# bharatlytics/faceRecognition_InfrenceEngine

Measured on AMD Instinct MI355X. Metric: faces/sec end-to-end @1080p, higher is better.
Workload: dtype f16

## Files before the change

### facerecognition_infrenceengine_amd/csrc/pnet_conv1.hip

```cpp
#include "detect_math.h"

namespace {

struct P1Args {
    const uint8_t* frames; int B, FH, FW;
    int H, W;
    const float* w;
    const float* bias; const float* slope;
    float* y;
    unsigned char* y_split;
    int Ho, Wo, Hp, Wp, regions_x, regions_y;
    const int32_t* list; const int32_t* list_count; int list_cap;
};

constexpr int P1_TW = 64, P1_IW = P1_TW + 2;
constexpr int P1_OCC = 3;
constexpr int P1_CTU = 4;
constexpr int P1_LEVEL_SHIFT = 27, P1_TILE_MASK = (1 << P1_LEVEL_SHIFT) - 1;

__device__ __forceinline__ float dpp_xor1(float v) {
    return __int_as_float(__builtin_amdgcn_update_dpp(0, __float_as_int(v), 0xB1, 0xf, 0xf, true));
}
__device__ __forceinline__ float dpp_shr1(float v) {
    return __int_as_float(__builtin_amdgcn_update_dpp(0, __float_as_int(v), 0x111, 0xf, 0xf, true));
}

template <int RPW, int RPB, bool F16, bool LIST>
__device__ __forceinline__ void pnet_conv1_body(const P1Args& a, const int item0, const int nitems) {
    constexpr int TH = 4 * RPW, IH = TH + 2, NPX = IH * P1_IW;
    constexpr int NPF = (NPX + 255) / 256;
    constexpr int NTAB = IH + P1_IW;
    constexpr int XPX = NPF * 256;
    static_assert(!F16 || XPX >= NPX + P1_IW + 4, "slack behind the tile for the zero-weight taps");
    constexpr int NXB = RPB > 1 ? 2 : 1, NTB = RPB > 1 ? 3 : 1;
    constexpr int XFL = F16 ? XPX * 4 : XPX * 3;
    __shared__ __attribute__((aligned(16))) float xin2[NXB][XFL];
    __shared__ __attribute__((aligned(16))) int4v tab[NTB][NTAB];
    const int tid = threadIdx.x, lane = tid & 63, wave = tid >> 6;
    const float pinf = opaque_inf();

    float wreg[6];
    half8 wfh[2], wfl[2];
    if constexpr (F16) {
#pragma unroll
        for (int st = 0; st < 2; ++st)
#pragma unroll
            for (int j = 0; j < 8; ++j) {
                const int kq_ = lane >> 4, kh = 2 * st + (kq_ >> 1), kw = (kq_ & 1) * 2 + (j >> 2), c = j & 3;
                const float w = (kh < 3 && kw < 3 && c < 3) ? a.w[((kh * 3 + kw) * 4 + c) * 16 + (lane & 15)] : 0.f;
                split_f16(w, wfh[st], wfl[st], j);
            }
    } else {
#pragma unroll
    for (int v = 0; v < 6; ++v) {
        const int c = v * 16 + (lane >> 2), r = lane & 3;
        float x = 0.f;
        if (c < 81) {
            const int k = c / 3, g = c - k * 3, tap = k / 3, ch = k - tap * 3;
            x = a.w[(tap * 4 + ch) * 16 + g * 4 + r];
        }
        wreg[v] = x;
    }
    }

    const int per_img = a.regions_x * a.regions_y;
    auto tile_of = [&](int item) { return LIST ? a.list[item] & P1_TILE_MASK : item; };
    const float ryr = (float)a.FH / (float)a.H, rxr = (float)a.FW / (float)a.W;
    const int frame_bytes = a.FH * a.FW * 3;

    auto make_tables = [&](int item, int buf) __attribute__((always_inline)) {
        if (tid < NTAB) {
            const int tile = tile_of(item);
            const int n = tile / per_img, rem = tile - n * per_img;
            const int ry = rem / a.regions_x, rx = rem - ry * a.regions_x;
            int4v e;
            if (tid < IH) {
                const int yy = ry * TH + tid;
                const Lerp l = lerp_coord(yy, ryr, a.FH);
                e = int4v{l.i0 * a.FW * 3, l.i1 * a.FW * 3, __float_as_int(l.w), yy < a.H ? 1 : 0};
            } else {
                const int xx = rx * P1_TW + (tid - IH);
                const Lerp l = lerp_coord(xx, rxr, a.FW);
                e = int4v{l.i0 * 3, __float_as_int(l.w), l.i1 != l.i0 ? 1 : 0, xx < a.W ? 1 : 0};
            }
            tab[buf][tid] = e;
        }
    };

    unsigned long long rq0[NPF], rq1[NPF];
    int rfl[NPF];
    int pos[NPF];
#pragma unroll
    for (int u = 0; u < NPF; ++u) {
        const int e = min(tid + u * 256, NPX - 1), iy = e / P1_IW;
        pos[u] = iy | ((IH + e - iy * P1_IW) << 16);
    }
    bool edge = true;
    auto load_tile = [&](int item, int buf) __attribute__((always_inline)) {
        const int n = tile_of(item) / per_img;
        const uint8_t* fbase = a.frames + (int64_t)n * frame_bytes;
        const bool last = n == a.B - 1;
        const int lim = frame_bytes - 8;
        int4v re[NPF], ce[NPF];
        bool special = false;
#pragma unroll
        for (int u = 0; u < NPF; ++u) { re[u] = tab[buf][pos[u] & 0xffff]; ce[u] = tab[buf][pos[u] >> 16]; }
#pragma unroll
        for (int u = 0; u < NPF; ++u) {
            const bool valid = (re[u][3] & ce[u][3]) != 0;
            const int o0 = valid ? re[u][0] + ce[u][0] : 0, o1 = valid ? re[u][1] + ce[u][0] : 0;
            int c0 = o0, c1 = o1, fl = ce[u][2];
            if (last) {
                c0 = min(o0, lim); c1 = min(o1, lim);
                fl |= ((o0 - c0) << 11) | ((o1 - c1) << 19);
            }
            rq0[u] = *reinterpret_cast<const u64_unaligned*>(fbase + c0);
            rq1[u] = *reinterpret_cast<const u64_unaligned*>(fbase + c1);
            rfl[u] = valid ? fl : -1;
            special = special || !valid || !(fl & 1);
        }
        edge = last || __builtin_amdgcn_ballot_w64(special) != 0;
    };
    auto store_tile_as = [&](int buf, float* xin, auto EDGE) __attribute__((always_inline)) {
        constexpr bool E = decltype(EDGE)::value;
        float wy[NPF], wx[NPF];
#pragma unroll
        for (int u = 0; u < NPF; ++u) {
            wy[u] = __int_as_float(tab[buf][pos[u] & 0xffff][2]);
            wx[u] = __int_as_float(tab[buf][pos[u] >> 16][1]);
        }
#pragma unroll
        for (int u = 0; u < NPF; ++u) {
            const int e = tid + u * 256;
            float v[3];
            const unsigned long long q0 = E ? rq0[u] >> ((rfl[u] >> 8) & 0xff) : rq0[u];
            const unsigned long long q1 = E ? rq1[u] >> ((rfl[u] >> 16) & 0xff) : rq1[u];
            const unsigned l0 = (unsigned)q0, h0 = (unsigned)(q0 >> 32), l1 = (unsigned)q1, h1 = (unsigned)(q1 >> 32);
            const bool two = !E || (rfl[u] & 1) != 0;
            const float a00[3] = {(float)((l0 >> 16) & 0xff), (float)((l0 >> 8) & 0xff), (float)(l0 & 0xff)};
            const float a01[3] = {(float)((h0 >> 8) & 0xff), (float)(h0 & 0xff), (float)(l0 >> 24)};
            const float a10[3] = {(float)((l1 >> 16) & 0xff), (float)((l1 >> 8) & 0xff), (float)(l1 & 0xff)};
            const float a11[3] = {(float)((h1 >> 8) & 0xff), (float)(h1 & 0xff), (float)(l1 >> 24)};
#pragma unroll
            for (int c = 0; c < 3; ++c) {
                const float sv = bilerp(a00[c], two ? a01[c] : a00[c], a10[c], two ? a11[c] : a10[c], wx[u], wy[u]);
                v[c] = (!E || rfl[u] >= 0) ? __builtin_fmaf(sv, 0.0078125f, -0.99609375f) : 0.f;
            }
            if constexpr (F16) {
                half4 hi, lo;
#pragma unroll
                for (int c = 0; c < 3; ++c) split_f16(v[c], hi, lo, c);
                hi[3] = lo[3] = (half_t)0.f;
                unsigned char* xz = reinterpret_cast<unsigned char*>(xin);
                *reinterpret_cast<half4*>(xz + e * 8) = hi;
                *reinterpret_cast<half4*>(xz + (XPX + e) * 8) = lo;
            } else {
                xin[e * 3 + 0] = v[0]; xin[e * 3 + 1] = v[1]; xin[e * 3 + 2] = v[2];
            }
        }
    };
    auto store_tile = [&](int buf, float* xdst) __attribute__((always_inline)) {
        if (edge) store_tile_as(buf, xdst, std::true_type{});
        else store_tile_as(buf, xdst, std::false_type{});
    };

    float4v bias_r[3], slope_r[3];
    bool mono = true;
#pragma unroll
    for (int g = 0; g < 3; ++g) {
        bias_r[g] = *reinterpret_cast<const float4v*>(a.bias + g * 4);
        slope_r[g] = *reinterpret_cast<const float4v*>(a.slope + g * 4);
#pragma unroll
        for (int e = 0; e < 4; ++e) mono = mono && slope_r[g][e] >= 0.f;
    }
    if (item0 < nitems) {
        make_tables(item0, 0);
        __syncthreads();
        load_tile(item0, 0);
        if (RPB > 1 && item0 + 1 < nitems) make_tables(item0 + 1, 1);
        if (RPB > 2 && item0 + 2 < nitems) make_tables(item0 + 2, 2);
        store_tile(0, xin2[0]);
    }
    __syncthreads();
    if (RPB > 1 && item0 + 1 < nitems) load_tile(item0 + 1, 1);

    for (int rr = 0; rr < RPB; ++rr) {
        const int item = item0 + rr;
        if (item >= nitems) break;
        const int tile_ = tile_of(item);
        const int n = tile_ / per_img, rem = tile_ - n * per_img;
        const int ry = rem / a.regions_x, rx = rem - ry * a.regions_x;
        const int y0 = ry * TH, x0 = rx * P1_TW;
        const float* xin = xin2[rr & (NXB - 1)];
        if constexpr (RPB > 1) {
            if (rr + 1 < RPB && item + 1 < nitems) store_tile((rr + 1) % 3, xin2[(rr + 1) & 1]);
            if (rr + 2 < RPB && item + 2 < nitems) load_tile(item + 2, (rr + 2) % 3);
            if (rr + 3 < RPB && item + 3 < nitems) make_tables(item + 3, rr % 3);
        }

        if constexpr (F16) {
            typedef half8 half8_a8 __attribute__((aligned(8)));
            const unsigned char* xz = reinterpret_cast<const unsigned char*>(xin);
            const int li = lane & 15, kq = lane >> 4;
            const float4v b4 = *reinterpret_cast<const float4v*>(a.bias + 4 * kq), s4 = *reinterpret_cast<const float4v*>(a.slope + 4 * kq);
            const int64_t fbase = (int64_t)n * a.Hp;
            auto conv16 = [&](int row, int ct) __attribute__((always_inline)) {
                const unsigned char* pb = xz + ((row + (kq >> 1)) * P1_IW + ct * 16 + li + 2 * (kq & 1)) * 8;
                const half8 h0 = *reinterpret_cast<const half8_a8*>(pb), l0 = *reinterpret_cast<const half8_a8*>(pb + XPX * 8);
                const half8 h1 = *reinterpret_cast<const half8_a8*>(pb + 2 * P1_IW * 8), l1 = *reinterpret_cast<const half8_a8*>(pb + (XPX + 2 * P1_IW) * 8);
                float4v q = {0.f, 0.f, 0.f, 0.f};
                q = __builtin_amdgcn_mfma_f32_16x16x32_f16(wfl[0], h0, q, 0, 0, 0);
                q = __builtin_amdgcn_mfma_f32_16x16x32_f16(wfh[0], l0, q, 0, 0, 0);
                q = __builtin_amdgcn_mfma_f32_16x16x32_f16(wfl[1], h1, q, 0, 0, 0);
                q = __builtin_amdgcn_mfma_f32_16x16x32_f16(wfh[1], l1, q, 0, 0, 0);
                q = __builtin_amdgcn_mfma_f32_16x16x32_f16(wfh[0], h0, q, 0, 0, 0);
                q = __builtin_amdgcn_mfma_f32_16x16x32_f16(wfh[1], h1, q, 0, 0, 0);
                return q;
            };
            auto put16 = [&](const float4v& m, int py, int px) __attribute__((always_inline)) {
                const int64_t pix = (fbase + py) * a.Wp + px;
                half4 hi, lo;
#pragma unroll
                for (int e = 0; e < 4; ++e) split_f16(m[e], hi, lo, e);
                const int2v hp = __builtin_bit_cast(int2v, hi), lp = __builtin_bit_cast(int2v, lo);
                const auto s0 = __builtin_amdgcn_permlane16_swap((unsigned)hp[0], (unsigned)lp[0], false, false);
                const auto s1 = __builtin_amdgcn_permlane16_swap((unsigned)hp[1], (unsigned)lp[1], false, false);
                *reinterpret_cast<int4v*>(a.y_split + pix * 64 + (kq & 1) * 32 + (kq >> 1) * 16) = int4v{(int)s0[0], (int)s1[0], (int)s0[1], (int)s1[1]};
                if (a.y && kq < 3) *reinterpret_cast<float4v*>(a.y + pix * 12 + 4 * kq) = m;
            };
            if (mono) {
                static_assert(RPW == 4 || !F16, "the packed epilogue pairs the wave's two row pairs");
                const bool interior = y0 + TH <= a.Ho && x0 + P1_TW <= a.Wo;
                float4v s4m, b4z;
#pragma unroll
                for (int e = 0; e < 4; ++e) { s4m[e] = 4 * kq + e < 10 ? s4[e] - 1.f : -1.f; b4z[e] = 4 * kq + e < 10 ? b4[e] : 0.f; }
                const int odd = li & 1;
                const int py = ((y0 + wave * RPW) >> 1) + odd;
#pragma unroll P1_CTU
                for (int ct = 0; ct < 4; ++ct) {
                    float4v m[2];
#pragma unroll
                    for (int rp = 0; rp < 2; ++rp) {
                        float4v d0 = conv16(wave * RPW + 2 * rp, ct), d1 = conv16(wave * RPW + 2 * rp + 1, ct);
                        if (!interior) {
                            const bool cin = x0 + ct * 16 + li < a.Wo;
                            const bool in0 = cin && y0 + wave * RPW + 2 * rp < a.Ho, in1 = cin && y0 + wave * RPW + 2 * rp + 1 < a.Ho;
#pragma unroll
                            for (int e = 0; e < 4; ++e) { d0[e] = in0 ? d0[e] : -INFINITY; d1[e] = in1 ? d1[e] : -INFINITY; }
                        }
#pragma unroll
                        for (int e = 0; e < 4; ++e) {
                            const float t = vmax(d0[e], d1[e], pinf);
                            m[rp][e] = vmax(t, dpp_xor1(t), pinf);
                        }
                    }
                    float4v v;
#pragma unroll
                    for (int e = 0; e < 4; ++e) {
                        float sh = dpp_shr1(m[1][e]);
                        asm volatile("" : "+v"(sh));
                        const float x = (odd ? sh : m[0][e]) + b4z[e];
                        v[e] = __builtin_fmaf(fminf(x, 0.f), s4m[e], x);
                    }
                    const int px = ((x0 + ct * 16) >> 1) + (li >> 1);
                    if (py < a.Hp && px < a.Wp) put16(v, py, px);
                }
            } else {
#pragma unroll
            for (int rp = 0; rp < RPW / 2; ++rp) {
#pragma unroll
                for (int ct = 0; ct < 4; ++ct) {
                    float4v d[2];
#pragma unroll
                    for (int h = 0; h < 2; ++h) {
                        const int row = wave * RPW + 2 * rp + h;
                        float4v q = conv16(row, ct);
                        q += b4;
#pragma unroll
                        for (int e = 0; e < 4; ++e) q[e] = q[e] > 0.f ? q[e] : q[e] * s4[e];
                        const bool inside = y0 + row < a.Ho && x0 + ct * 16 + li < a.Wo;
                        d[h] = inside ? q : float4v{-INFINITY, -INFINITY, -INFINITY, -INFINITY};
                    }
                    float4v m;
#pragma unroll
                    for (int e = 0; e < 4; ++e) {
                        const float t = vmax(d[0][e], d[1][e], pinf);
                        m[e] = 4 * kq + e < 10 ? vmax(t, dpp_xor1(t), pinf) : 0.f;
                    }
                    const int py = (y0 + wave * RPW + 2 * rp) >> 1, px = (x0 + ct * 16 + li) >> 1;
                    if ((li & 1) == 0 && py < a.Hp && px < a.Wp) put16(m, py, px);
                }
            }
            }
        } else {
        float4v acc[RPW][3];
#pragma unroll
        for (int r = 0; r < RPW; ++r)
#pragma unroll
            for (int g = 0; g < 3; ++g) acc[r][g] = float4v{0.f, 0.f, 0.f, 0.f};
        const float* xb = xin + ((wave * RPW) * P1_IW + lane) * 3;
        static_for<RPW + 2>([&](auto IR) {
            constexpr int ir = decltype(IR)::value;
            float xv[9];
#pragma unroll
            for (int q = 0; q < 9; ++q) xv[q] = xb[ir * P1_IW * 3 + q];
            static_for<9>([&](auto Q) {
                constexpr int q = decltype(Q)::value;
                static_for<3>([&](auto KH) {
                    constexpr int kh = decltype(KH)::value, r = ir - kh;
                    if constexpr (r >= 0 && r < RPW) {
                        static_for<3>([&](auto G) {
                            constexpr int g = decltype(G)::value;
                            constexpr int c = (kh * 9 + q) * 3 + g;
                            acc[r][g] = __builtin_amdgcn_mfma_f32_4x4x1f32(wreg[c / 16], xv[q], acc[r][g], 4, c % 16, 0);
                        });
                    }
                });
            });
        });

        const int xcol = x0 + lane;
        const bool interior = y0 + TH <= a.Ho && x0 + P1_TW <= a.Wo;
        auto put = [&](const float4v (&pv)[3], int py, int px) __attribute__((always_inline)) {
            const int64_t pix = ((int64_t)n * a.Hp + py) * a.Wp + px;
            float* o = a.y + pix * 12;
#pragma unroll
            for (int g = 0; g < 3; ++g) *reinterpret_cast<float4v*>(o + g * 4) = pv[g];
            if (a.y_split) {
                half8 hi[2], lo[2];
#pragma unroll
                for (int c = 0; c < 16; ++c) split_f16(c < 10 ? pv[c >> 2][c & 3] : 0.f, hi[c >> 3], lo[c >> 3], c & 7);
                unsigned char* o2 = a.y_split + pix * 64;
                *reinterpret_cast<half8*>(o2) = hi[0];
                *reinterpret_cast<half8*>(o2 + 16) = hi[1];
                *reinterpret_cast<half8*>(o2 + 32) = lo[0];
                *reinterpret_cast<half8*>(o2 + 48) = lo[1];
            }
        };
        if (mono) {
            if (!interior) {
#pragma unroll
                for (int r = 0; r < RPW; ++r) {
                    const bool inside = y0 + wave * RPW + r < a.Ho && xcol < a.Wo;
#pragma unroll
                    for (int g = 0; g < 3; ++g)
                        acc[r][g] = inside ? acc[r][g] : float4v{-INFINITY, -INFINITY, -INFINITY, -INFINITY};
                }
            }
            float4v pv[RPW / 2][3];
#pragma unroll
            for (int rp = 0; rp < RPW / 2; ++rp)
#pragma unroll
                for (int g = 0; g < 3; ++g)
#pragma unroll
                    for (int e = 0; e < 4; ++e) {
                        const float m = vmax(acc[2 * rp][g][e], acc[2 * rp + 1][g][e], pinf);
                        pv[rp][g][e] = vmax(m, dpp_xor1(m), pinf);
                    }
            float4v q[3];
            int py = (y0 + wave * RPW) >> 1;
            bool writer = (lane & 1) == 0;
            if constexpr (RPW == 4) {
#pragma unroll
                for (int g = 0; g < 3; ++g)
#pragma unroll
                    for (int e = 0; e < 4; ++e) {
                        const float t = dpp_shr1(pv[1][g][e]);
                        q[g][e] = (lane & 1) ? t : pv[0][g][e];
                    }
                py += lane & 1;
                writer = true;
            } else {
#pragma unroll
                for (int g = 0; g < 3; ++g) q[g] = pv[0][g];
            }
#pragma unroll
            for (int g = 0; g < 3; ++g) {
                q[g] += bias_r[g];
#pragma unroll
                for (int e = 0; e < 4; ++e) q[g][e] = q[g][e] > 0.f ? q[g][e] : q[g][e] * slope_r[g][e];
            }
            const int px = (x0 >> 1) + (lane >> 1);
            if (writer && py < a.Hp && px < a.Wp) put(q, py, px);
        } else {
#pragma unroll
            for (int r = 0; r < RPW; ++r) {
                const bool inside = y0 + wave * RPW + r < a.Ho && xcol < a.Wo;
#pragma unroll
                for (int g = 0; g < 3; ++g) {
                    float4v v = acc[r][g] + bias_r[g];
#pragma unroll
                    for (int e = 0; e < 4; ++e) v[e] = v[e] > 0.f ? v[e] : v[e] * slope_r[g][e];
                    acc[r][g] = inside ? v : float4v{-INFINITY, -INFINITY, -INFINITY, -INFINITY};
                }
            }
#pragma unroll
            for (int rp = 0; rp < RPW / 2; ++rp) {
                float4v pv[3];
#pragma unroll
                for (int g = 0; g < 3; ++g)
#pragma unroll
                    for (int e = 0; e < 4; ++e) {
                        const float m = vmax(acc[2 * rp][g][e], acc[2 * rp + 1][g][e], pinf);
                        pv[g][e] = vmax(m, dpp_xor1(m), pinf);
                    }
                const int py = (y0 + wave * RPW + 2 * rp) >> 1, px = xcol >> 1;
                if ((lane & 1) == 0 && py < a.Hp && px < a.Wp) put(pv, py, px);
            }
        }
        }
        if (rr + 1 < RPB && item + 1 < nitems) __syncthreads();
    }
}

template <int RPW, int RPB, bool F16 = false, bool LIST = false>
__global__ __launch_bounds__(256, RPW == 4 ? (F16 ? P1_OCC : 3) : 6) void pnet_conv1_kernel(P1Args a) {
    const int nitems = LIST ? min(*a.list_count, a.list_cap) : a.regions_x * a.regions_y * a.B;
    pnet_conv1_body<RPW, RPB, F16, LIST>(a, blockIdx.x * RPB, nitems);
}

#define P1_MAXL 16
struct P1Levels {
    float* y[P1_MAXL]; unsigned char* y_split[P1_MAXL];
    int H[P1_MAXL], W[P1_MAXL], rpb[P1_MAXL], first[P1_MAXL + 1];
    int nlevels;
};
template <int RPW, int RPB, bool F16 = false, bool LIST = false>
__global__ __launch_bounds__(256, RPW == 4 ? (F16 ? P1_OCC : 3) : 6) void pnet_conv1_levels(P1Args a, P1Levels t) {
    int l = 0, item0 = blockIdx.x, nitems = 0;
    if constexpr (LIST) {
        if (item0 >= min(*a.list_count, a.list_cap)) return;
        l = min((int)((unsigned)a.list[item0] >> P1_LEVEL_SHIFT), t.nlevels - 1);
        nitems = item0 + 1;
    } else {
        while (l + 1 < t.nlevels && (int)blockIdx.x >= t.first[l + 1]) ++l;
    }
    a.H = t.H[l]; a.W = t.W[l]; a.y = t.y[l]; a.y_split = t.y_split[l];
    a.Ho = a.H - 2; a.Wo = a.W - 2; a.Hp = (a.Ho + 1) / 2; a.Wp = (a.Wo + 1) / 2;
    a.regions_x = (a.Wo + P1_TW - 1) / P1_TW; a.regions_y = (a.Ho + 4 * RPW - 1) / (4 * RPW);
    if constexpr (!LIST) {
        item0 = ((int)blockIdx.x - t.first[l]) * t.rpb[l];
        nitems = min(a.regions_x * a.regions_y * a.B, item0 + t.rpb[l]);
    }
    pnet_conv1_body<RPW, RPB, F16, LIST>(a, item0, nitems);
}

template <int RPW, int RPB, bool F16 = false, bool LIST = false>
int launch_p1(P1Args a, hipStream_t s) {
    constexpr int TH = 4 * RPW;
    a.regions_x = (a.Wo + P1_TW - 1) / P1_TW;
    a.regions_y = (a.Ho + TH - 1) / TH;
    const int64_t nitems = LIST ? a.list_cap : (int64_t)a.regions_x * a.regions_y * a.B;
    if (nitems >= (LIST ? 1ll << P1_LEVEL_SHIFT : 1ll << 31)) return FR_E_INVALID;
    pnet_conv1_kernel<RPW, RPB, F16, LIST><<<(unsigned)((nitems + RPB - 1) / RPB), 256, 0, s>>>(a);
    return FR_OK;
}

}

int fr_pnet_conv1_launch(const uint8_t* frames, int B, int FH, int FW, int H, int W, const float* w, const float* bias,
                         const float* slope, float* y, void* y_split, hipStream_t s) {
    P1Args a{frames, B, FH, FW, H, W, w, bias, slope, y, (unsigned char*)y_split, H - 2, W - 2, 0, 0, 0, 0, nullptr, nullptr, 0};
    a.Hp = (a.Ho + 1) / 2; a.Wp = (a.Wo + 1) / 2;
    const int64_t tiles16 = (int64_t)((a.Ho + 15) / 16) * ((a.Wo + P1_TW - 1) / P1_TW) * B;
    if (tiles16 >= 4096) return launch_p1<4, 8>(a, s);
    if (tiles16 >= 512) return launch_p1<4, 1>(a, s);
    return launch_p1<2, 1>(a, s);
}

extern "C" int fr_pnet_conv1_band(int mode, const uint8_t* frames, int B, int FH, int FW, int H, int W, const float* w,
                                  const float* bias, const float* slope, float* y, void* y_split, const int32_t* list,
                                  const int32_t* list_count, int list_cap, fr_stream_t stream) {
    FR_REQUIRE(frames && w && bias && slope && B > 0 && FH > 0 && FW > 0 && H >= 3 && W >= 3, "fr_pnet_conv1_band: bad argument");
    P1Args a{frames, B, FH, FW, H, W, w, bias, slope, y, (unsigned char*)y_split, H - 2, W - 2, 0, 0, 0, 0, list, list_count, list_cap};
    a.Hp = (a.Ho + 1) / 2; a.Wp = (a.Wo + 1) / 2;
    hipStream_t s = fr_stream(stream);
    int rc;
    if (mode == 0) {
        FR_REQUIRE(y_split, "fr_pnet_conv1_band: mode 0 writes the split map");
        const int64_t tiles16 = (int64_t)((a.Ho + 15) / 16) * ((a.Wo + P1_TW - 1) / P1_TW) * B;
        rc = tiles16 >= 4096 ? launch_p1<4, 8, true>(a, s) : launch_p1<4, 1, true>(a, s);
    } else if (mode == 1) {
        FR_REQUIRE(y && list && list_count && list_cap > 0, "fr_pnet_conv1_band: mode 1 needs the f32 map and a tile list");
        rc = launch_p1<4, 1, false, true>(a, s);
    } else { FR_REQUIRE(false, "fr_pnet_conv1_band: mode must be 0 or 1"); }
    if (rc != FR_OK) { fr_set_error("fr_pnet_conv1_band: too many tiles"); return rc; }
    FR_CHECK_LAUNCH("pnet_conv1_kernel (band)");
    return FR_OK;
}

extern "C" int fr_pnet_pyramid_conv1(int mode, const uint8_t* frames, int B, int FH, int FW, const fr_pnet_level* levels, int nlevels,
                                     const float* w, const float* bias, const float* slope, const int32_t* list,
                                     const int32_t* list_count, int list_cap, fr_stream_t stream) {
    FR_REQUIRE(frames && w && bias && slope && levels && B > 0 && FH > 0 && FW > 0 && nlevels > 0 && nlevels <= P1_MAXL,
               "fr_pnet_pyramid_conv1: bad argument (1 .. %d levels)", P1_MAXL);
    FR_REQUIRE(mode == 0 || mode == 1, "fr_pnet_pyramid_conv1: mode must be 0 or 1");
    for (int l = 0; l < nlevels; ++l) {
        const fr_pnet_level& L = levels[l];
        FR_REQUIRE(L.x1 && L.x1s && L.hs >= 3 && L.ws >= 3 && L.H1 == (L.hs - 1) / 2 && L.W1 == (L.ws - 1) / 2,
                   "fr_pnet_pyramid_conv1: level %d: bad entry", l);
        FR_REQUIRE((int64_t)B * ((L.hs + 13) / 16) * ((L.ws + 61) / 64) < (1ll << P1_LEVEL_SHIFT), "fr_pnet_pyramid_conv1: level %d: too many tiles", l);
    }
    P1Args a{frames, B, FH, FW, 0, 0, w, bias, slope, nullptr, nullptr, 0, 0, 0, 0, 0, 0, list, list_count, list_cap};
    hipStream_t s = fr_stream(stream);
    if (mode == 1) {
        FR_REQUIRE(list && list_count && list_cap > 0, "fr_pnet_pyramid_conv1: mode 1 needs a tile list");
        P1Levels t{};
        t.nlevels = nlevels;
        for (int l = 0; l < nlevels; ++l) {
            t.y[l] = const_cast<float*>(levels[l].x1); t.y_split[l] = nullptr; t.H[l] = levels[l].hs; t.W[l] = levels[l].ws; t.rpb[l] = 1;
        }
        pnet_conv1_levels<4, 1, false, true><<<(unsigned)list_cap, 256, 0, s>>>(a, t);
        FR_CHECK_LAUNCH("pnet_conv1_levels (tile list)");
        return FR_OK;
    }
    for (int form = 1; form >= 0; --form) {
        P1Levels t{};
        int64_t total = 0;
        for (int l = 0; l < nlevels; ++l) {
            const fr_pnet_level& L = levels[l];
            if ((L.f16 != 0) != (form != 0)) continue;
            const int k = t.nlevels++;
            t.y[k] = form ? nullptr : const_cast<float*>(L.x1); t.y_split[k] = reinterpret_cast<unsigned char*>(L.x1s);
            t.H[k] = L.hs; t.W[k] = L.ws;
            const int64_t tiles = (int64_t)B * ((L.hs + 13) / 16) * ((L.ws + 61) / 64);
            t.rpb[k] = tiles >= 4096 ? 8 : 1;
            t.first[k] = (int)total;
            total += (tiles + t.rpb[k] - 1) / t.rpb[k];
        }
        if (!t.nlevels) continue;
        FR_REQUIRE(total < (1ll << 31), "fr_pnet_pyramid_conv1: too many tiles");
        t.first[t.nlevels] = (int)total;
        if (form) pnet_conv1_levels<4, 8, true><<<(unsigned)total, 256, 0, s>>>(a, t);
        else pnet_conv1_levels<4, 8><<<(unsigned)total, 256, 0, s>>>(a, t);
        FR_CHECK_LAUNCH("pnet_conv1_levels");
    }
    return FR_OK;
}
```

Before: 26690.

## Use buffer stores, shared epilogue params, and specialize tile loop on steady/mono

Replaces the global stores of the pooled maps with raw buffer stores that take 32-bit offsets. Out-of-range lanes are redirected past the end of the buffer instead of being guarded by branches, and 64-bit address arithmetic is dropped. Bias and slope epilogue vectors are precomputed once into shared memory, and the tile loop is split into a steady-state part with fewer bounds checks. The mono path becomes a compile-time template instead of a runtime branch. A VIEW template variant writes the f32 map only when it is requested, at lower occupancy; the change also adds a guard that rejects maps of 4 GB or more.

After: 26770, median of 3. Within noise of the previous version (+0.3%).

```diff
diff --git a/facerecognition_infrenceengine_amd/csrc/pnet_conv1.hip b/facerecognition_infrenceengine_amd/csrc/pnet_conv1.hip
--- a/facerecognition_infrenceengine_amd/csrc/pnet_conv1.hip
+++ b/facerecognition_infrenceengine_amd/csrc/pnet_conv1.hip
@@ -25,8 +25,9 @@
     return __int_as_float(__builtin_amdgcn_update_dpp(0, __float_as_int(v), 0x111, 0xf, 0xf, true));
 }
 
-template <int RPW, int RPB, bool F16, bool LIST>
+template <int RPW, int RPB, bool F16, bool LIST, bool VIEW = false>
 __device__ __forceinline__ void pnet_conv1_body(const P1Args& a, const int item0, const int nitems) {
+    static_assert(F16 || !VIEW, "the f32 form always writes the f32 map");
     constexpr int TH = 4 * RPW, IH = TH + 2, NPX = IH * P1_IW;
     constexpr int NPF = (NPX + 255) / 256;
     constexpr int NTAB = IH + P1_IW;
@@ -36,8 +37,26 @@
     constexpr int XFL = F16 ? XPX * 4 : XPX * 3;
     __shared__ __attribute__((aligned(16))) float xin2[NXB][XFL];
     __shared__ __attribute__((aligned(16))) int4v tab[NTB][NTAB];
+    __shared__ __attribute__((aligned(16))) float4v prm[F16 ? 4 : 1][4];
     const int tid = threadIdx.x, lane = tid & 63, wave = tid >> 6;
     const float pinf = opaque_inf();
+    if constexpr (F16) {
+        if (tid < 16) {
+            const int kind = tid >> 2, q = tid & 3;
+            const float4v b = *reinterpret_cast<const float4v*>(a.bias + 4 * q), sl = *reinterpret_cast<const float4v*>(a.slope + 4 * q);
+            float4v v;
+#pragma unroll
+            for (int e = 0; e < 4; ++e) {
+                const bool real = 4 * q + e < 10;
+                v[e] = kind == 0 ? b[e] : kind == 1 ? sl[e] : kind == 2 ? (real ? b[e] : 0.f) : (real ? sl[e] - 1.f : -1.f);
+            }
+            prm[kind][q] = v;
+        }
+    }
+    typedef unsigned uint4v __attribute__((ext_vector_type(4)));
+    const unsigned npool = (unsigned)a.B * (unsigned)a.Hp * (unsigned)a.Wp;
+    const unsigned y_bytes = a.y ? npool * 48u : 0u, ys_bytes = a.y_split ? npool * 64u : 0u;
+    const __amdgpu_buffer_rsrc_t yrs = buffer_rsrc(a.y, y_bytes), srs = buffer_rsrc(a.y_split, ys_bytes);
 
     float wreg[6];
     half8 wfh[2], wfl[2];
@@ -149,7 +168,11 @@
             if constexpr (F16) {
                 half4 hi, lo;
 #pragma unroll
-                for (int c = 0; c < 3; ++c) split_f16(v[c], hi, lo, c);
+                for (int c = 0; c < 3; ++c) {
+                    float x = v[c];
+                    asm("" : "+v"(x));
+                    split_f16(x, hi, lo, c);
+                }
                 hi[3] = lo[3] = (half_t)0.f;
                 unsigned char* xz = reinterpret_cast<unsigned char*>(xin);
                 *reinterpret_cast<half4*>(xz + e * 8) = hi;
@@ -183,27 +206,27 @@
     }
     __syncthreads();
     if (RPB > 1 && item0 + 1 < nitems) load_tile(item0 + 1, 1);
-
-    for (int rr = 0; rr < RPB; ++rr) {
+    const int ntile = min(nitems - item0, RPB);
+
+    auto tile_step = [&](const int rr, auto STEADY_, auto MONO_) __attribute__((always_inline)) {
+        constexpr bool STEADY = decltype(STEADY_)::value, MONO = decltype(MONO_)::value;
         const int item = item0 + rr;
-        if (item >= nitems) break;
         const int tile_ = tile_of(item);
         const int n = tile_ / per_img, rem = tile_ - n * per_img;
         const int ry = rem / a.regions_x, rx = rem - ry * a.regions_x;
         const int y0 = ry * TH, x0 = rx * P1_TW;
         const float* xin = xin2[rr & (NXB - 1)];
         if constexpr (RPB > 1) {
-            if (rr + 1 < RPB && item + 1 < nitems) store_tile((rr + 1) % 3, xin2[(rr + 1) & 1]);
-            if (rr + 2 < RPB && item + 2 < nitems) load_tile(item + 2, (rr + 2) % 3);
-            if (rr + 3 < RPB && item + 3 < nitems) make_tables(item + 3, rr % 3);
+            if (STEADY || rr + 1 < ntile) store_tile((rr + 1) % 3, xin2[(rr + 1) & 1]);
+            if (STEADY || rr + 2 < ntile) load_tile(item + 2, (rr + 2) % 3);
+            if (STEADY || rr + 3 < ntile) make_tables(item + 3, rr % 3);
         }
 
         if constexpr (F16) {
             typedef half8 half8_a8 __attribute__((aligned(8)));
             const unsigned char* xz = reinterpret_cast<const unsigned char*>(xin);
             const int li = lane & 15, kq = lane >> 4;
-            const float4v b4 = *reinterpret_cast<const float4v*>(a.bias + 4 * kq), s4 = *reinterpret_cast<const float4v*>(a.slope + 4 * kq);
-            const int64_t fbase = (int64_t)n * a.Hp;
+            const unsigned fbase = (unsigned)n * (unsigned)a.Hp;
             auto conv16 = [&](int row, int ct) __attribute__((always_inline)) {
                 const unsigned char* pb = xz + ((row + (kq >> 1)) * P1_IW + ct * 16 + li + 2 * (kq & 1)) * 8;
                 const half8 h0 = *reinterpret_cast<const half8_a8*>(pb), l0 = *reinterpret_cast<const half8_a8*>(pb + XPX * 8);
@@ -217,23 +240,22 @@
                 q = __builtin_amdgcn_mfma_f32_16x16x32_f16(wfh[1], h1, q, 0, 0, 0);
                 return q;
             };
-            auto put16 = [&](const float4v& m, int py, int px) __attribute__((always_inline)) {
-                const int64_t pix = (fbase + py) * a.Wp + px;
+            auto put16 = [&](const float4v& m, int py, int px, bool ok) __attribute__((always_inline)) {
+                const unsigned pix = (fbase + (unsigned)py) * (unsigned)a.Wp + (unsigned)px;
                 half4 hi, lo;
 #pragma unroll
                 for (int e = 0; e < 4; ++e) split_f16(m[e], hi, lo, e);
                 const int2v hp = __builtin_bit_cast(int2v, hi), lp = __builtin_bit_cast(int2v, lo);
                 const auto s0 = __builtin_amdgcn_permlane16_swap((unsigned)hp[0], (unsigned)lp[0], false, false);
                 const auto s1 = __builtin_amdgcn_permlane16_swap((unsigned)hp[1], (unsigned)lp[1], false, false);
-                *reinterpret_cast<int4v*>(a.y_split + pix * 64 + (kq & 1) * 32 + (kq >> 1) * 16) = int4v{(int)s0[0], (int)s1[0], (int)s0[1], (int)s1[1]};
-                if (a.y && kq < 3) *reinterpret_cast<float4v*>(a.y + pix * 12 + 4 * kq) = m;
+                __builtin_amdgcn_raw_buffer_store_b128(uint4v{s0[0], s1[0], s0[1], s1[1]}, srs, ok ? pix * 64u + (kq & 1) * 32 + (kq >> 1) * 16 : ys_bytes, 0, 0);
+                if constexpr (VIEW)
+                    __builtin_amdgcn_raw_buffer_store_b128(__builtin_bit_cast(uint4v, m), yrs, ok && kq < 3 ? pix * 48u + 16 * kq : y_bytes, 0, 0);
             };
-            if (mono) {
+            if constexpr (MONO) {
                 static_assert(RPW == 4 || !F16, "the packed epilogue pairs the wave's two row pairs");
                 const bool interior = y0 + TH <= a.Ho && x0 + P1_TW <= a.Wo;
-                float4v s4m, b4z;
-#pragma unroll
-                for (int e = 0; e < 4; ++e) { s4m[e] = 4 * kq + e < 10 ? s4[e] - 1.f : -1.f; b4z[e] = 4 * kq + e < 10 ? b4[e] : 0.f; }
+                const float4v b4z = prm[2][kq], s4m = prm[3][kq];
                 const int odd = li & 1;
                 const int py = ((y0 + wave * RPW) >> 1) + odd;
 #pragma unroll P1_CTU
@@ -263,9 +285,10 @@
                         v[e] = __builtin_fmaf(fminf(x, 0.f), s4m[e], x);
                     }
                     const int px = ((x0 + ct * 16) >> 1) + (li >> 1);
-                    if (py < a.Hp && px < a.Wp) put16(v, py, px);
+                    put16(v, py, px, py < a.Hp && px < a.Wp);
                 }
             } else {
+            const float4v b4 = prm[0][kq], s4 = prm[1][kq];
 #pragma unroll
             for (int rp = 0; rp < RPW / 2; ++rp) {
 #pragma unroll
@@ -288,7 +311,7 @@
                         m[e] = 4 * kq + e < 10 ? vmax(t, dpp_xor1(t), pinf) : 0.f;
                     }
                     const int py = (y0 + wave * RPW + 2 * rp) >> 1, px = (x0 + ct * 16 + li) >> 1;
-                    if ((li & 1) == 0 && py < a.Hp && px < a.Wp) put16(m, py, px);
+                    put16(m, py, px, (li & 1) == 0 && py < a.Hp && px < a.Wp);
                 }
             }
             }
@@ -321,23 +344,23 @@
 
         const int xcol = x0 + lane;
         const bool interior = y0 + TH <= a.Ho && x0 + P1_TW <= a.Wo;
-        auto put = [&](const float4v (&pv)[3], int py, int px) __attribute__((always_inline)) {
-            const int64_t pix = ((int64_t)n * a.Hp + py) * a.Wp + px;
-            float* o = a.y + pix * 12;
-#pragma unroll
-            for (int g = 0; g < 3; ++g) *reinterpret_cast<float4v*>(o + g * 4) = pv[g];
-            if (a.y_split) {
+        auto put = [&](const float4v (&pv)[3], int py, int px, bool ok) __attribute__((always_inline)) {
+            const unsigned pix = ((unsigned)n * (unsigned)a.Hp + (unsigned)py) * (unsigned)a.Wp + (unsigned)px;
+            const unsigned o = ok ? pix * 48u : y_bytes;
+#pragma unroll
+            for (int g = 0; g < 3; ++g) __builtin_amdgcn_raw_buffer_store_b128(__builtin_bit_cast(uint4v, pv[g]), yrs, o + g * 16, 0, 0);
+            if (!LIST || a.y_split) {
                 half8 hi[2], lo[2];
 #pragma unroll
                 for (int c = 0; c < 16; ++c) split_f16(c < 10 ? pv[c >> 2][c & 3] : 0.f, hi[c >> 3], lo[c >> 3], c & 7);
-                unsigned char* o2 = a.y_split + pix * 64;
-                *reinterpret_cast<half8*>(o2) = hi[0];
-                *reinterpret_cast<half8*>(o2 + 16) = hi[1];
-                *reinterpret_cast<half8*>(o2 + 32) = lo[0];
-                *reinterpret_cast<half8*>(o2 + 48) = lo[1];
+                const unsigned o2 = ok ? pix * 64u : ys_bytes;
+                __builtin_amdgcn_raw_buffer_store_b128(__builtin_bit_cast(uint4v, hi[0]), srs, o2, 0, 0);
+                __builtin_amdgcn_raw_buffer_store_b128(__builtin_bit_cast(uint4v, hi[1]), srs, o2 + 16, 0, 0);
+                __builtin_amdgcn_raw_buffer_store_b128(__builtin_bit_cast(uint4v, lo[0]), srs, o2 + 32, 0, 0);
+                __builtin_amdgcn_raw_buffer_store_b128(__builtin_bit_cast(uint4v, lo[1]), srs, o2 + 48, 0, 0);
             }
         };
-        if (mono) {
+        if constexpr (MONO) {
             if (!interior) {
 #pragma unroll
                 for (int r = 0; r < RPW; ++r) {
@@ -381,7 +404,7 @@
                 for (int e = 0; e < 4; ++e) q[g][e] = q[g][e] > 0.f ? q[g][e] : q[g][e] * slope_r[g][e];
             }
             const int px = (x0 >> 1) + (lane >> 1);
-            if (writer && py < a.Hp && px < a.Wp) put(q, py, px);
+            put(q, py, px, writer && py < a.Hp && px < a.Wp);
         } else {
 #pragma unroll
             for (int r = 0; r < RPW; ++r) {
@@ -405,18 +428,26 @@
                         pv[g][e] = vmax(m, dpp_xor1(m), pinf);
                     }
                 const int py = (y0 + wave * RPW + 2 * rp) >> 1, px = xcol >> 1;
-                if ((lane & 1) == 0 && py < a.Hp && px < a.Wp) put(pv, py, px);
-            }
-        }
-        }
-        if (rr + 1 < RPB && item + 1 < nitems) __syncthreads();
-    }
-}
-
-template <int RPW, int RPB, bool F16 = false, bool LIST = false>
-__global__ __launch_bounds__(256, RPW == 4 ? (F16 ? P1_OCC : 3) : 6) void pnet_conv1_kernel(P1Args a) {
+                put(pv, py, px, (lane & 1) == 0 && py < a.Hp && px < a.Wp);
+            }
+        }
+        }
+        if (STEADY || rr + 1 < ntile) __syncthreads();
+    };
+    auto walk = [&](auto MONO_) __attribute__((always_inline)) {
+        int rr = 0;
+        if constexpr (RPB > 3 && F16)
+            for (; rr + 3 < ntile; ++rr) tile_step(rr, std::true_type{}, MONO_);
+        for (; rr < ntile; ++rr) tile_step(rr, std::false_type{}, MONO_);
+    };
+    if (mono) walk(std::true_type{});
+    else walk(std::false_type{});
+}
+
+template <int RPW, int RPB, bool F16 = false, bool LIST = false, bool VIEW = false>
+__global__ __launch_bounds__(256, RPW == 4 ? (F16 ? (VIEW ? 2 : P1_OCC) : 3) : 6) void pnet_conv1_kernel(P1Args a) {
     const int nitems = LIST ? min(*a.list_count, a.list_cap) : a.regions_x * a.regions_y * a.B;
-    pnet_conv1_body<RPW, RPB, F16, LIST>(a, blockIdx.x * RPB, nitems);
+    pnet_conv1_body<RPW, RPB, F16, LIST, VIEW>(a, blockIdx.x * RPB, nitems);
 }
 
 #define P1_MAXL 16
@@ -445,14 +476,17 @@
     pnet_conv1_body<RPW, RPB, F16, LIST>(a, item0, nitems);
 }
 
-template <int RPW, int RPB, bool F16 = false, bool LIST = false>
+constexpr bool p1_map_fits(int64_t B, int64_t Hp, int64_t Wp) { return B * Hp * Wp * 64 <= 0xffffffffll - 64; }
+
+template <int RPW, int RPB, bool F16 = false, bool LIST = false, bool VIEW = false>
 int launch_p1(P1Args a, hipStream_t s) {
     constexpr int TH = 4 * RPW;
+    if (!p1_map_fits(a.B, a.Hp, a.Wp)) return FR_E_INVALID;
     a.regions_x = (a.Wo + P1_TW - 1) / P1_TW;
     a.regions_y = (a.Ho + TH - 1) / TH;
     const int64_t nitems = LIST ? a.list_cap : (int64_t)a.regions_x * a.regions_y * a.B;
     if (nitems >= (LIST ? 1ll << P1_LEVEL_SHIFT : 1ll << 31)) return FR_E_INVALID;
-    pnet_conv1_kernel<RPW, RPB, F16, LIST><<<(unsigned)((nitems + RPB - 1) / RPB), 256, 0, s>>>(a);
+    pnet_conv1_kernel<RPW, RPB, F16, LIST, VIEW><<<(unsigned)((nitems + RPB - 1) / RPB), 256, 0, s>>>(a);
     return FR_OK;
 }
 
@@ -479,12 +513,13 @@
     if (mode == 0) {
         FR_REQUIRE(y_split, "fr_pnet_conv1_band: mode 0 writes the split map");
         const int64_t tiles16 = (int64_t)((a.Ho + 15) / 16) * ((a.Wo + P1_TW - 1) / P1_TW) * B;
-        rc = tiles16 >= 4096 ? launch_p1<4, 8, true>(a, s) : launch_p1<4, 1, true>(a, s);
+        if (y) rc = tiles16 >= 4096 ? launch_p1<4, 8, true, false, true>(a, s) : launch_p1<4, 1, true, false, true>(a, s);
+        else rc = tiles16 >= 4096 ? launch_p1<4, 8, true>(a, s) : launch_p1<4, 1, true>(a, s);
     } else if (mode == 1) {
         FR_REQUIRE(y && list && list_count && list_cap > 0, "fr_pnet_conv1_band: mode 1 needs the f32 map and a tile list");
         rc = launch_p1<4, 1, false, true>(a, s);
     } else { FR_REQUIRE(false, "fr_pnet_conv1_band: mode must be 0 or 1"); }
-    if (rc != FR_OK) { fr_set_error("fr_pnet_conv1_band: too many tiles"); return rc; }
+    if (rc != FR_OK) { fr_set_error("fr_pnet_conv1_band: too many tiles, or a level map of 4 GB or more"); return rc; }
     FR_CHECK_LAUNCH("pnet_conv1_kernel (band)");
     return FR_OK;
 }
@@ -500,6 +535,7 @@
         FR_REQUIRE(L.x1 && L.x1s && L.hs >= 3 && L.ws >= 3 && L.H1 == (L.hs - 1) / 2 && L.W1 == (L.ws - 1) / 2,
                    "fr_pnet_pyramid_conv1: level %d: bad entry", l);
         FR_REQUIRE((int64_t)B * ((L.hs + 13) / 16) * ((L.ws + 61) / 64) < (1ll << P1_LEVEL_SHIFT), "fr_pnet_pyramid_conv1: level %d: too many tiles", l);
+        FR_REQUIRE(p1_map_fits(B, L.H1, L.W1), "fr_pnet_pyramid_conv1: level %d: a map of 4 GB or more", l);
     }
     P1Args a{frames, B, FH, FW, 0, 0, w, bias, slope, nullptr, nullptr, 0, 0, 0, 0, 0, 0, list, list_count, list_cap};
     hipStream_t s = fr_stream(stream);
```
